# Shaibk/Matrix-FHE-GPU

Hardware: AMD Instinct MI355X
Metric: forward-NTT/s (N=2^16, L RNS limbs) (higher is better)
Workload: dtype u64; 1 GPU; batched forward negacyclic NTT (phantom convention), N=2^16, L=8 x 50-bit primes, batch=1024 per GPU; N=65536, limbs=8, batch_per_gpu=1024, arith=f64, parallelism=residue-batch shard x1 (no collective)

## Files before the change

matrix-fhe-gpu_amd/csrc/ntt_kernels.hpp:

```cpp
#pragma once
#include <type_traits>

#include "ntt_arith.hpp"

#ifndef MFHE_NTT_CPOL_IN
#define MFHE_NTT_CPOL_IN 0
#endif
#ifndef MFHE_NTT_CPOL_OUT
#define MFHE_NTT_CPOL_OUT 18
#endif
#ifndef MFHE_NTT_CPOL_MID_LD
#define MFHE_NTT_CPOL_MID_LD 0
#endif
#ifndef MFHE_NTT_CPOL_MID_ST
#define MFHE_NTT_CPOL_MID_ST 0
#endif
#ifndef MFHE_NTT_U64_INV_TWPRE
#define MFHE_NTT_U64_INV_TWPRE 1
#endif
#ifndef MFHE_NTT_COL_DMA
#define MFHE_NTT_COL_DMA 1
#endif

namespace mfhe {

struct TwSrcF {
    const double* p;
    __device__ __forceinline__ double get(size_t i) const { return p[i]; }
};
struct TwSrcU {
    const uint64_t* w;
    const uint64_t* ws;
    __device__ __forceinline__ ulonglong2 get(size_t i) const {
#ifdef MFHE_EXP_TWCONST
        return make_ulonglong2((uint64_t)i * 0x9E3779B97F4A7C15ull >> 6, (uint64_t)i * 0xC2B2AE3D27D4EB4Full);
#endif
        return make_ulonglong2(w[i], ws[i]);
    }
};

template <class TS>
struct PassArgs {
    uint64_t* data;
    TS tw;
    TS twist;
    TS ninv;
    const LimbConst* limbs;
    const uint64_t* qraw;
    int qstride;
    uint64_t batch;
    int nl, start_limb;
    int logN, s0;
    uint32_t nblocks;
};

__device__ __forceinline__ uint32_t xcd_remap(uint32_t b, uint32_t nb) {
    const uint32_t q = nb >> 3, r = nb & 7, x = b & 7, s = b >> 3;
    return (x < r ? x * (q + 1) : r * (q + 1) + (x - r) * q) + s;
}

template <int LOG_G, int LOG_R>
struct Geo {
    static constexpr int G = 1 << LOG_G;
    static constexpr int R = 1 << LOG_R;
    static constexpr int TG = G / R;
    static constexpr int NR = (LOG_G + LOG_R - 1) / LOG_R;
    static constexpr int GS = G + G / 16 + 1;
    __host__ __device__ static constexpr int HB(int r) { return LOG_G - 1 - r * LOG_R; }
    __host__ __device__ static constexpr int WL(int r) { return (HB(r) - LOG_R + 1) > 0 ? (HB(r) - LOG_R + 1) : 0; }
    __device__ __forceinline__ static uint32_t g_of(int r, uint32_t tau, uint32_t k) {
        const int wl = WL(r);
        return ((tau >> wl) << (wl + LOG_R)) | (k << wl) | (tau & ((1u << wl) - 1));
    }
    __device__ __forceinline__ static uint32_t pad(uint32_t g) { return g + (g >> 4); }
};

__device__ __forceinline__ uint32_t brev_bits(uint32_t x, int bits) { return __brev(x) >> (32 - bits); }

template <int I, int N, class F>
__device__ __forceinline__ void static_for(F&& f) {
    if constexpr (I < N) {
        f(std::integral_constant<int, I>{});
        static_for<I + 1, N>(f);
    }
}

template <int R, int BB, bool LAST, class A, class T, class TWF>
__device__ __forceinline__ void u60_inv_stage(const A& ar, T (&x)[R], TWF&& tw, typename A::Tw wn) {
    constexpr int half = 1 << BB;
    static_for<0, R>([&](auto kc) {
        constexpr int k = decltype(kc)::value;
        if constexpr (!(k & half)) {
            constexpr int e0 = U60InvBounds<R>::after(k, BB);
            constexpr int e = e0 == 3 ? 0 : e0;
            if constexpr (e0 == 3) {
                x[k] = ar.template red<3>(x[k]);
                x[k + half] = ar.template red<3>(x[k + half]);
            }
            const auto w = tw(k);
            ar.template gs_b<e>(x[k], x[k + half], w);
            if constexpr (LAST) x[k] = ar.mulmod(x[k], wn);
        }
    });
}

template <class A>
__device__ __forceinline__ uint64_t inv_out(const A& ar, typename A::T x) {
    if constexpr (kLazyU60<A>) return ar.canon_inv(x);
    else return ar.canon(x);
}

template <int R, int N, class A, class T>
__device__ __forceinline__ void u60_inv_round_end(const A& ar, T (&x)[R]) {
    static_for<0, R>([&](auto kc) {
        constexpr int k = decltype(kc)::value;
        x[k] = ar.template red<U60InvBounds<R>::after(k, N)>(x[k]);
    });
}

struct TileLoc {
    uint64_t* base;
    size_t twoff;
    uint32_t off0;
    uint64_t hi;
    int mod;
    bool active;
};

template <int LOG_G, int NG, bool COLS, bool UNI>
__device__ __forceinline__ TileLoc tile_loc(uint64_t* data, uint64_t batch, int nl, int start_limb, int logN, int s0,
                                            uint32_t lb, uint32_t gl) {
    const int logS = logN - s0 - LOG_G;
    const int log_gpp = logS + s0;
    const uint32_t npl = (uint32_t)(batch * (uint64_t)nl);
    uint32_t v;
    uint64_t hi, lo;
    if constexpr (COLS) {
        constexpr int LOG_NG = __builtin_ctz(NG);
        const int log_tpp = log_gpp - LOG_NG, log_ct = logS - LOG_NG;
        v = lb >> log_tpp;
        const uint32_t tile = lb & ((1u << log_tpp) - 1);
        hi = tile >> log_ct;
        lo = ((uint64_t)(tile & ((1u << log_ct) - 1)) << LOG_NG) + gl;
    } else if constexpr (UNI) {
        const uint64_t g0 = (uint64_t)lb * NG;
        v = (uint32_t)(g0 >> log_gpp);
        const uint64_t rem = (g0 & ((1ull << log_gpp) - 1)) + gl;
        hi = rem >> logS;
        lo = rem & ((1ull << logS) - 1);
    } else {
        const uint64_t gid = (uint64_t)lb * NG + gl;
        v = (uint32_t)(gid >> log_gpp);
        const uint64_t rem = gid & ((1ull << log_gpp) - 1);
        hi = rem >> logS;
        lo = rem & ((1ull << logS) - 1);
    }
    TileLoc t;
    t.active = v < npl;
    if (!t.active) v = 0;
    const uint32_t bt = (uint32_t)batch;
    const int l = (int)(v / bt);
    const uint64_t b = v - (uint32_t)l * bt;
    t.mod = start_limb + l;
    t.base = data + ((b * (uint64_t)nl + (uint64_t)l) << logN);
    t.twoff = (size_t)t.mod << logN;
    t.hi = hi;
    t.off0 = (uint32_t)((hi << (logN - s0)) | lo);
    return t;
}

constexpr int kPackUnitBytes = 1664;
constexpr int kPackRowBytes = 2048;

template <class A, class TS, int LOG_G, int LOG_R, int NG, bool COLS, bool INV, bool IN_RAW, bool OUT_RAW,
          bool TWIST, bool BREV, bool UNI, bool PACK = false>
struct NttPass {
    static_assert(!PACK || (LOG_G == 8 && LOG_R == 4 && NG == 16 && UNI && !INV && !TWIST && !BREV &&
                            (COLS ? (OUT_RAW && !IN_RAW) : (IN_RAW && !OUT_RAW))),
                  "PACK: forward N = 2^16 two-pass plan only");
    static constexpr bool COL_DMA = MFHE_NTT_COL_DMA && COLS && !INV && !IN_RAW && UNI && !TWIST &&
                                    (1 << LOG_G) * NG * 8 == 32768 && NG % 2 == 0;
    static constexpr bool PACK_OUT = PACK && COLS;
    static constexpr bool PACK_IN = PACK && !COLS;
    using Gm = Geo<LOG_G, LOG_R>;
    using T = typename A::T;
    using Tw = typename A::Tw;
    static constexpr int R = Gm::R, TG = Gm::TG, NR = Gm::NR, GS = Gm::GS;
    static constexpr int NT = NG * TG;
    static constexpr size_t LDS_BYTES = (NR > 1 || BREV) ? (size_t)NG * GS * sizeof(uint64_t) : 0;
    static constexpr int r_load = (INV && COLS) ? (NR - 1) : 0;
    static constexpr int r_store = (!INV && COLS) ? (NR - 1) : 0;

    const PassArgs<TS>& a;
    uint32_t gl, tau;
    int s0, logS;

    __device__ __forceinline__ explicit NttPass(const PassArgs<TS>& args) : a(args) {
        const uint32_t t = threadIdx.x;
        gl = COLS ? (t % NG) : (t / TG);
        tau = COLS ? (t / NG) : (t % TG);
        s0 = COLS ? 0 : a.logN - LOG_G;
        logS = a.logN - s0 - LOG_G;
    }
    __device__ __forceinline__ uint32_t jidx(const TileLoc& L, uint32_t g) const { return L.off0 | (g << logS); }
    __device__ __forceinline__ TileLoc locate(uint32_t lb) const {
        return tile_loc<LOG_G, NG, COLS, UNI>(a.data, a.batch, a.nl, a.start_limb, a.logN, s0, lb, gl);
    }
    static constexpr int kCpolLd = IN_RAW ? MFHE_NTT_CPOL_MID_LD : MFHE_NTT_CPOL_IN;
    static constexpr int kCpolSt = OUT_RAW ? MFHE_NTT_CPOL_MID_ST : MFHE_NTT_CPOL_OUT;

    __device__ __forceinline__ void load(const TileLoc& L, uint64_t (&raw)[R]) const {
        if constexpr (COL_DMA) return;
        if constexpr (PACK_IN) {
            const uint32_t rb = (uint32_t)(L.hi >> 4);
            const char* base = (const char*)L.base + (size_t)(16 * rb) * kPackRowBytes;
#pragma unroll
            for (int s = 0; s < 7; ++s) {
                const uint32_t q = threadIdx.x + NT * s;
                ulonglong2 v = make_ulonglong2(0, 0);
                if (s < 6 || q < 16 * kPackUnitBytes / 16) {
                    const uint32_t t = q / 104, w = q - 104 * t;
                    v = *(const ulonglong2*)(base + (w >> 3) * kPackRowBytes + t * 128 + (w & 7) * 16);
                }
                raw[2 * s] = v.x;
                raw[2 * s + 1] = v.y;
            }
            return;
        }
        if constexpr (UNI && kCpolLd != 0) {
            const __amdgpu_buffer_rsrc_t rs = __builtin_amdgcn_make_buffer_rsrc(L.base, 0, 0x7FFFFFFF, 0x00020000);
#pragma unroll
            for (int k = 0; k < R; ++k)
                raw[k] = __builtin_bit_cast(uint64_t, __builtin_amdgcn_raw_buffer_load_b64(
                                                          rs, (int)(jidx(L, Gm::g_of(r_load, tau, k)) * 8u), 0, kCpolLd));
        } else {
#pragma unroll
            for (int k = 0; k < R; ++k) {
#ifdef MFHE_EXP_SKIP
                if (IN_RAW && k >= 12) { raw[k] = 0; continue; }
#endif
                raw[k] = L.base[jidx(L, Gm::g_of(r_load, tau, k))];
            }
        }
    }

    __device__ __forceinline__ void compute_store(const TileLoc& L, const uint64_t (&raw)[R], uint64_t* lds) const {
        uint64_t* my_lds = lds + (size_t)gl * GS;
        LimbConst lc;
        if (a.limbs) {
            lc = a.limbs[L.mod];
        } else {
            lc.q = a.qraw[(size_t)L.mod * a.qstride];
            lc.qf = (double)lc.q;
            lc.qinv = 1.0 / lc.qf;
        }
        const A ar(lc);
        const size_t twoff = L.twoff;
        const uint32_t tau_ = tau;

        T x[R];
        if constexpr (COL_DMA) {
            typedef __attribute__((address_space(3))) void* lds_vp;
            constexpr int CPR = NG / 2;
            const uint32_t w = threadIdx.x >> 6, lane = threadIdx.x & 63;
            const char* tile = (const char*)(L.base + (L.off0 - gl));
            __syncthreads();
#pragma unroll
            for (int i = 0; i < 32768 / (NT * 16); ++i) {
                const uint32_t q = (i * (NT / 64) + w) * 64 + lane;
                const char* src = tile + (size_t)(q / CPR) * ((size_t)8 << (a.logN - LOG_G)) + (q % CPR) * 16;
                __builtin_amdgcn_global_load_lds((const void*)src,
                                                 (lds_vp)((char*)lds + (size_t)(i * (NT / 64) + w) * 1024), 16, 0,
                                                 kCpolLd);
            }
            asm volatile("s_waitcnt vmcnt(0)" ::: "memory");
            __syncthreads();
#pragma unroll
            for (int k = 0; k < R; ++k) x[k] = A::from_u64(lds[(size_t)Gm::g_of(r_load, tau_, k) * NG + gl]);
        } else if constexpr (PACK_IN) {
            __syncthreads();
            ulonglong2* img = (ulonglong2*)lds;
#pragma unroll
            for (int s = 0; s < 7; ++s) {
                const uint32_t q = threadIdx.x + NT * s;
                if (s < 6 || q < 16 * kPackUnitBytes / 16) img[q] = make_ulonglong2(raw[2 * s], raw[2 * s + 1]);
            }
            __syncthreads();
            const uint32_t C = threadIdx.x, t = C >> 4, c = C & 15;
            const char* ub = (const char*)lds + t * kPackUnitBytes;
            uint64_t w[13];
#pragma unroll
            for (int s = 0; s < 4; ++s) {
                const ulonglong2 v = *(const ulonglong2*)(ub + c * 64 + 16 * s);
                w[2 * s] = v.x;
                w[2 * s + 1] = v.y;
            }
#pragma unroll
            for (int s = 0; s < 2; ++s) {
                const ulonglong2 v = *(const ulonglong2*)(ub + 1024 + c * 32 + 16 * s);
                w[8 + 2 * s] = v.x;
                w[9 + 2 * s] = v.y;
            }
            w[12] = *(const uint32_t*)(ub + 1536 + c * 4);
            __syncthreads();
#pragma unroll
            for (int i = 0; i < 16; ++i) {
                const uint64_t lo = (w[i >> 1] >> (32 * (i & 1))) & 0xFFFFFFFFull;
                const uint64_t mid = (w[8 + (i >> 2)] >> (16 * (i & 3))) & 0xFFFFull;
                const uint64_t top = (w[12] >> (2 * i)) & 3ull;
                lds[(size_t)i * GS + Gm::pad(C)] = lo | (mid << 32) | (top << 48);
            }
            __syncthreads();
#pragma unroll
            for (int k = 0; k < R; ++k) x[k] = A::from_u64(my_lds[Gm::pad(Gm::g_of(0, tau_, k))]);
        } else {
#pragma unroll
            for (int k = 0; k < R; ++k) {
                x[k] = IN_RAW ? A::from_raw(raw[k]) : A::from_u64(raw[k]);
                if constexpr (TWIST && !INV) x[k] = ar.mulmod(x[k], a.twist.get(twoff + jidx(L, Gm::g_of(r_load, tau_, k))));
            }
        }

        auto exchange = [&](auto rf, auto rt, bool brev_pos) {
            constexpr int r_from = decltype(rf)::value, r_to = decltype(rt)::value;
            __syncthreads();
#pragma unroll
            for (int k = 0; k < R; ++k) {
                uint32_t g = Gm::g_of(r_from, tau_, k);
                if (brev_pos) g = brev_bits(g, LOG_G);
                my_lds[Gm::pad(g)] = A::to_raw(x[k]);
            }
            __syncthreads();
#pragma unroll
            for (int k = 0; k < R; ++k) x[k] = A::from_raw(my_lds[Gm::pad(Gm::g_of(r_to, tau_, k))]);
        };

        constexpr bool kTwPre = INV && !COLS && kIsU64<A> && MFHE_NTT_U64_INV_TWPRE;
        Tw wpre[kTwPre ? R / 2 : 1];
        if constexpr (kTwPre) {
            constexpr int r = NR - 1, wl = Gm::WL(r), bit = wl;
            const int s = s0 + (LOG_G - 1 - bit);
            const uint64_t twb = twoff + (1ull << s) + (L.hi << (LOG_G - 1 - bit)) + ((uint64_t)(tau_ >> wl) << (LOG_R - 1));
#pragma unroll
            for (int m = 0; m < R / 2; ++m) wpre[m] = a.tw.get(twb + (uint64_t)m);
        }
        if constexpr (INV && !COLS && (NR > 1 || BREV))
            exchange(std::integral_constant<int, 0>{}, std::integral_constant<int, NR - 1>{}, BREV);

        auto stage = [&](auto rc, auto bc) {
            constexpr int r = decltype(rc)::value, bb = decltype(bc)::value;
            constexpr int hb = Gm::HB(r), wl = Gm::WL(r);
            constexpr int bit = wl + bb;
            if constexpr (bit <= hb) {
                const int s = s0 + (LOG_G - 1 - bit);
                constexpr int half = 1 << bb;
                const uint64_t tau_hi = tau_ >> wl;
                const uint64_t twb =
                    twoff + (1ull << s) + (L.hi << (LOG_G - 1 - bit)) + (tau_hi << (LOG_R - 1 - bb));
                if constexpr (!INV) {
                    constexpr int fb = (LOG_R - 1 < hb - wl) ? LOG_R - 1 : hb - wl;
                    constexpr bool first = bb == fb && (r > 0 || IN_RAW);
                    static_assert(!kLazyU60<A> || LOG_R <= 4, "U60 bound: at most 4 stages between reductions");
#pragma unroll
                    for (int k = 0; k < R; ++k) {
                        if (k & half) continue;
                        const Tw w = a.tw.get(twb + (uint64_t)(k >> (bb + 1)));
                        if constexpr (first) ar.ct_first(x[k], x[k + half], w);
                        else ar.ct(x[k], x[k + half], w);
                    }
                } else {
                    constexpr int ri = NR - 1 - r;
                    constexpr int first = (Gm::HB(NR - 1) < LOG_R - 1 ? Gm::HB(NR - 1) : LOG_R - 1) + 1;
                    constexpr int e = ri == 0 ? bb : first + (ri - 1) * LOG_R + bb;
                    if constexpr (kLazyU60<A>) {
                        if (s == 0) {
                            const Tw wn = a.ninv.get((size_t)L.mod);
                            const Tw w1 = a.tw.get(twoff + 1);
                            u60_inv_stage<R, bb, true>(ar, x, [&](int) { return w1; }, wn);
                        } else {
                            u60_inv_stage<R, bb, false>(ar, x, [&](int k) {
                                if constexpr (kTwPre && r == NR - 1 && bb == 0) return wpre[k >> 1];
                                else return a.tw.get(twb + (uint64_t)(k >> (bb + 1)));
                            }, Tw{});
                        }
                    } else if (s == 0) {
                        const Tw wn = a.ninv.get((size_t)L.mod);
                        const Tw w1 = a.tw.get(twoff + 1);
#pragma unroll
                        for (int k = 0; k < R; ++k) {
                            if (k & half) continue;
                            T u = x[k], vv = x[k + half];
                            ar.gs_lazy(u, vv, w1);
                            x[k] = ar.mulmod(u, wn);
                            x[k + half] = vv;
                        }
                    } else {
#pragma unroll
                        for (int k = 0; k < R; ++k) {
                            if (k & half) continue;
                            Tw w;
                            if constexpr (kTwPre && r == NR - 1 && bb == 0) w = wpre[k >> 1];
                            else w = a.tw.get(twb + (uint64_t)(k >> (bb + 1)));
                            if constexpr (e % 2 == 0) ar.gs_lazy(x[k], x[k + half], w);
                            else ar.gs(x[k], x[k + half], w);
                        }
                    }
                }
            }
        };

        if constexpr (!INV) {
            static_for<0, NR>([&](auto rc) {
                constexpr int r = decltype(rc)::value;
                if constexpr (r > 0) {
                    exchange(std::integral_constant<int, r - 1>{}, rc, false);
#pragma unroll
                    for (int k = 0; k < R; ++k) x[k] = ar.round_reduce(x[k]);
                }
                static_for<0, LOG_R>([&](auto bi) {
                    stage(rc, std::integral_constant<int, LOG_R - 1 - decltype(bi)::value>{});
                });
            });
        } else {
            static_for<0, NR>([&](auto ri) {
                constexpr int r = NR - 1 - decltype(ri)::value;
                if constexpr (r < NR - 1)
                    exchange(std::integral_constant<int, r + 1>{}, std::integral_constant<int, r>{}, false);
                static_for<0, LOG_R>([&](auto bi) { stage(std::integral_constant<int, r>{}, bi); });
                if constexpr (kLazyU60<A>) {
                    constexpr int hb = Gm::HB(r), wl = Gm::WL(r);
                    constexpr int nexec = (hb - wl + 1) < LOG_R ? (hb - wl + 1) : LOG_R;
                    if constexpr (r > 0 || OUT_RAW) u60_inv_round_end<R, nexec>(ar, x);
                }
            });
        }

        if constexpr (!INV && !COLS && (NR > 1 || BREV))
            exchange(std::integral_constant<int, NR - 1>{}, std::integral_constant<int, 0>{}, BREV);
        if constexpr (PACK_OUT) {
            uint32_t lo[16], mid[8] = {}, top = 0;
#pragma unroll
            for (int k = 0; k < 16; ++k) {
                const uint64_t u = ar.canon(x[k]);
                lo[k] = (uint32_t)u;
                const uint32_t hi = (uint32_t)(u >> 32);
                mid[k >> 1] |= (hi & 0xFFFFu) << (16 * (k & 1));
                top |= (hi >> 16) << (2 * k);
            }
            __syncthreads();
            char* ub = (char*)lds + tau_ * kPackUnitBytes;
            uint4* plo = (uint4*)(ub + gl * 64);
            uint4* pmid = (uint4*)(ub + 1024 + gl * 32);
#pragma unroll
            for (int s = 0; s < 4; ++s) plo[s] = make_uint4(lo[4 * s], lo[4 * s + 1], lo[4 * s + 2], lo[4 * s + 3]);
#pragma unroll
            for (int s = 0; s < 2; ++s) pmid[s] = make_uint4(mid[4 * s], mid[4 * s + 1], mid[4 * s + 2], mid[4 * s + 3]);
            *(uint32_t*)(ub + 1536 + gl * 4) = top;
            __syncthreads();
            if (L.active) {
                const uint4* src = (const uint4*)lds;
                char* dst = (char*)L.base + (size_t)(L.off0 & ~15u) * 8;
                for (uint32_t q = threadIdx.x; q < 16 * kPackUnitBytes / 16; q += NT) {
                    const uint32_t m = q >> 3, rb = m / 13, j = m - 13 * rb;
                    *(uint4*)(dst + (size_t)(16 * rb + j) * kPackRowBytes + (q & 7) * 16) = src[q];
                }
            }
            return;
        }
        if (L.active) {
            if constexpr (UNI && kCpolSt != 0) {
                const __amdgpu_buffer_rsrc_t rs = __builtin_amdgcn_make_buffer_rsrc(L.base, 0, 0x7FFFFFFF, 0x00020000);
#pragma unroll
                for (int k = 0; k < R; ++k) {
                    const uint32_t g = Gm::g_of(r_store, tau_, k);
                    T y = x[k];
                    if constexpr (TWIST && INV) y = ar.mulmod(y, a.twist.get(twoff + jidx(L, g)));
                    const uint64_t o = OUT_RAW ? ar.raw_out(y) : INV ? inv_out(ar, y) : ar.canon(y);
                    __builtin_amdgcn_raw_buffer_store_b64(__builtin_bit_cast(__attribute__((ext_vector_type(2))) unsigned, o),
                                                          rs, (int)(jidx(L, g) * 8u), 0, kCpolSt);
                }
            } else {
#pragma unroll
                for (int k = 0; k < R; ++k) {
                    const uint32_t g = Gm::g_of(r_store, tau_, k);
                    T y = x[k];
                    if constexpr (TWIST && INV) y = ar.mulmod(y, a.twist.get(twoff + jidx(L, g)));
#ifdef MFHE_EXP_SKIP
                    if (OUT_RAW && k >= 12) continue;
#endif
                    L.base[jidx(L, g)] = OUT_RAW ? ar.raw_out(y) : INV ? inv_out(ar, y) : ar.canon(y);
                }
            }
        }
    }
};

template <class P, bool PF, class TS>
__device__ __forceinline__ void pass_loop(const PassArgs<TS>& a, uint64_t* lds) {
    const P p(a);
    const uint32_t nb = a.nblocks;
    uint32_t lt = blockIdx.x;
    if (lt >= nb) return;
    TileLoc L = p.locate(xcd_remap(lt, nb));
    uint64_t raw[P::R];
    p.load(L, raw);
    while (true) {
        const uint32_t nlt = lt + gridDim.x;
        const bool more = nlt < nb;
        TileLoc Ln;
        uint64_t nraw[PF ? P::R : 1];
        if constexpr (PF) {
            if (more) {
                Ln = p.locate(xcd_remap(nlt, nb));
                p.load(Ln, nraw);
            }
        }
        p.compute_store(L, raw, lds);
        if (!more) break;
        lt = nlt;
        if constexpr (PF) {
            L = Ln;
            for (int k = 0; k < P::R; ++k) raw[k] = nraw[k];
        } else {
            L = p.locate(xcd_remap(lt, nb));
            p.load(L, raw);
        }
    }
}

#ifndef MFHE_NTT_MIN_WG_CU
#define MFHE_NTT_MIN_WG_CU 1
#endif
constexpr int min_waves_per_simd(int nt) {
    return (MFHE_NTT_MIN_WG_CU * nt / 256) < 1 ? 1 : (MFHE_NTT_MIN_WG_CU * nt / 256);
}

#ifndef MFHE_NTT_U64_BLOCK_W4
#define MFHE_NTT_U64_BLOCK_W4 0
#endif
template <class A, bool COLS>
constexpr int pass_min_waves(int nt) {
    return (MFHE_NTT_U64_BLOCK_W4 && kIsU64<A> && !COLS && nt <= 256) ? 4 : min_waves_per_simd(nt);
}

template <class A, class TS, int LOG_G, int LOG_R, int NG, bool COLS, bool INV, bool IN_RAW, bool OUT_RAW,
          bool TWIST, bool BREV, bool UNI, bool PF, bool PACK = false>
__global__ __launch_bounds__(NG * (1 << (LOG_G - LOG_R)), (pass_min_waves<A, COLS>(NG * (1 << (LOG_G - LOG_R)))))
void ntt_pass_kernel(PassArgs<TS> a) {
    extern __shared__ __attribute__((aligned(16))) uint64_t lds[];
    pass_loop<NttPass<A, TS, LOG_G, LOG_R, NG, COLS, INV, IN_RAW, OUT_RAW, TWIST, BREV, UNI, PACK>, PF>(a, lds);
}

}
```

Before: 2.849 million NTT/s.

## Prefetch per-round twiddles before LDS exchange and use lighter LDS-only barriers

Generalises the inverse-only twiddle prefetch so that, in the row (block) pass, the twiddles for up to four stages of the next radix round are loaded into registers before the shared-memory exchange. Global twiddle latency can then overlap the exchange barrier. It also swaps __syncthreads in the row-pass exchange for an inline s_waitcnt lgkmcnt(0) plus s_barrier, or only a waitcnt when the block fits in one wavefront, which skips waiting on outstanding global memory operations. The costs are higher register pressure from the prefetch array and correctness that now depends on hand-written barrier semantics.

New measurement: 2.864 million NTT/s (median of 6 runs). No clear change (+0.6%).

```diff
diff --git a/matrix-fhe-gpu_amd/csrc/ntt_kernels.hpp b/matrix-fhe-gpu_amd/csrc/ntt_kernels.hpp
--- a/matrix-fhe-gpu_amd/csrc/ntt_kernels.hpp
+++ b/matrix-fhe-gpu_amd/csrc/ntt_kernels.hpp
@@ -17,6 +17,15 @@
 #endif
 #ifndef MFHE_NTT_U64_INV_TWPRE
 #define MFHE_NTT_U64_INV_TWPRE 1
+#endif
+#ifndef MFHE_NTT_U64_BLOCK_TWPRE
+#define MFHE_NTT_U64_BLOCK_TWPRE 4
+#endif
+#ifndef MFHE_NTT_F64_BLOCK_TWPRE
+#define MFHE_NTT_F64_BLOCK_TWPRE 4
+#endif
+#ifndef MFHE_NTT_BLOCK_LDS_SYNC
+#define MFHE_NTT_BLOCK_LDS_SYNC 1
 #endif
 #ifndef MFHE_NTT_COL_DMA
 #define MFHE_NTT_COL_DMA 1
@@ -191,6 +200,29 @@
     static constexpr int r_load = (INV && COLS) ? (NR - 1) : 0;
     static constexpr int r_store = (!INV && COLS) ? (NR - 1) : 0;
 
+    static constexpr bool LDS_ONLY_SYNC = !COLS && MFHE_NTT_BLOCK_LDS_SYNC;
+    __device__ __forceinline__ static void lds_sync_before_write() {
+        if constexpr (!LDS_ONLY_SYNC) __syncthreads();
+        else if constexpr (NT <= 64) asm volatile("" ::: "memory");
+        else asm volatile("s_waitcnt lgkmcnt(0)\n\ts_barrier" ::: "memory");
+    }
+    __device__ __forceinline__ static void lds_sync_before_read() {
+        if constexpr (!LDS_ONLY_SYNC) __syncthreads();
+        else if constexpr (NT <= 64) asm volatile("s_waitcnt lgkmcnt(0)" ::: "memory");
+        else asm volatile("s_waitcnt lgkmcnt(0)\n\ts_barrier" ::: "memory");
+    }
+
+    static constexpr bool BLOCK = !COLS && (INV ? OUT_RAW : IN_RAW);
+    static constexpr int TWPRE = !BLOCK ? 0 : kIsU64<A> ? MFHE_NTT_U64_BLOCK_TWPRE : MFHE_NTT_F64_BLOCK_TWPRE;
+    static constexpr int TWPRE_ENTRY = (INV && !COLS && kIsU64<A> && MFHE_NTT_U64_INV_TWPRE && TWPRE < 1) ? 1 : TWPRE;
+    __host__ __device__ static constexpr int nexec(int r) {
+        return (Gm::HB(r) - Gm::WL(r) + 1) < LOG_R ? (Gm::HB(r) - Gm::WL(r) + 1) : LOG_R;
+    }
+    __host__ __device__ static constexpr bool tw_pre(int r, int bb) {
+        const int n = INV ? (r == NR - 1 ? TWPRE_ENTRY : TWPRE) : (r > 0 ? TWPRE : 0);
+        return bb < nexec(r) && (INV ? bb : nexec(r) - 1 - bb) < n;
+    }
+
     const PassArgs<TS>& a;
     uint32_t gl, tau;
     int s0, logS;
@@ -323,27 +355,36 @@
 
         auto exchange = [&](auto rf, auto rt, bool brev_pos) {
             constexpr int r_from = decltype(rf)::value, r_to = decltype(rt)::value;
-            __syncthreads();
+            lds_sync_before_write();
 #pragma unroll
             for (int k = 0; k < R; ++k) {
                 uint32_t g = Gm::g_of(r_from, tau_, k);
                 if (brev_pos) g = brev_bits(g, LOG_G);
                 my_lds[Gm::pad(g)] = A::to_raw(x[k]);
             }
-            __syncthreads();
+            lds_sync_before_read();
 #pragma unroll
             for (int k = 0; k < R; ++k) x[k] = A::from_raw(my_lds[Gm::pad(Gm::g_of(r_to, tau_, k))]);
         };
 
-        constexpr bool kTwPre = INV && !COLS && kIsU64<A> && MFHE_NTT_U64_INV_TWPRE;
-        Tw wpre[kTwPre ? R / 2 : 1];
-        if constexpr (kTwPre) {
-            constexpr int r = NR - 1, wl = Gm::WL(r), bit = wl;
+        auto tw_base = [&](auto rc, auto bc) -> uint64_t {
+            constexpr int r = decltype(rc)::value, bb = decltype(bc)::value;
+            constexpr int wl = Gm::WL(r), bit = wl + bb;
             const int s = s0 + (LOG_G - 1 - bit);
-            const uint64_t twb = twoff + (1ull << s) + (L.hi << (LOG_G - 1 - bit)) + ((uint64_t)(tau_ >> wl) << (LOG_R - 1));
-#pragma unroll
-            for (int m = 0; m < R / 2; ++m) wpre[m] = a.tw.get(twb + (uint64_t)m);
-        }
+            return twoff + (1ull << s) + (L.hi << (LOG_G - 1 - bit)) + ((uint64_t)(tau_ >> wl) << (LOG_R - 1 - bb));
+        };
+        Tw wp[LOG_R][R / 2];
+        auto tw_prefetch = [&](auto rc) {
+            static_for<0, LOG_R>([&](auto bc) {
+                constexpr int r = decltype(rc)::value, bb = decltype(bc)::value;
+                if constexpr (tw_pre(r, bb)) {
+                    const uint64_t twb = tw_base(rc, bc);
+#pragma unroll
+                    for (int m = 0; m < (R >> (bb + 1)); ++m) wp[bb][m] = a.tw.get(twb + (uint64_t)m);
+                }
+            });
+        };
+        if constexpr (INV) tw_prefetch(std::integral_constant<int, NR - 1>{});
         if constexpr (INV && !COLS && (NR > 1 || BREV))
             exchange(std::integral_constant<int, 0>{}, std::integral_constant<int, NR - 1>{}, BREV);
 
@@ -354,9 +395,11 @@
             if constexpr (bit <= hb) {
                 const int s = s0 + (LOG_G - 1 - bit);
                 constexpr int half = 1 << bb;
-                const uint64_t tau_hi = tau_ >> wl;
-                const uint64_t twb =
-                    twoff + (1ull << s) + (L.hi << (LOG_G - 1 - bit)) + (tau_hi << (LOG_R - 1 - bb));
+                const uint64_t twb = tw_base(rc, bc);
+                auto tw_at = [&](int m) -> Tw {
+                    if constexpr (tw_pre(r, bb)) return wp[bb][m];
+                    else return a.tw.get(twb + (uint64_t)m);
+                };
                 if constexpr (!INV) {
                     constexpr int fb = (LOG_R - 1 < hb - wl) ? LOG_R - 1 : hb - wl;
                     constexpr bool first = bb == fb && (r > 0 || IN_RAW);
@@ -364,7 +407,7 @@
 #pragma unroll
                     for (int k = 0; k < R; ++k) {
                         if (k & half) continue;
-                        const Tw w = a.tw.get(twb + (uint64_t)(k >> (bb + 1)));
+                        const Tw w = tw_at(k >> (bb + 1));
                         if constexpr (first) ar.ct_first(x[k], x[k + half], w);
                         else ar.ct(x[k], x[k + half], w);
                     }
@@ -378,10 +421,7 @@
                             const Tw w1 = a.tw.get(twoff + 1);
                             u60_inv_stage<R, bb, true>(ar, x, [&](int) { return w1; }, wn);
                         } else {
-                            u60_inv_stage<R, bb, false>(ar, x, [&](int k) {
-                                if constexpr (kTwPre && r == NR - 1 && bb == 0) return wpre[k >> 1];
-                                else return a.tw.get(twb + (uint64_t)(k >> (bb + 1)));
-                            }, Tw{});
+                            u60_inv_stage<R, bb, false>(ar, x, [&](int k) { return tw_at(k >> (bb + 1)); }, Tw{});
                         }
                     } else if (s == 0) {
                         const Tw wn = a.ninv.get((size_t)L.mod);
@@ -398,9 +438,7 @@
 #pragma unroll
                         for (int k = 0; k < R; ++k) {
                             if (k & half) continue;
-                            Tw w;
-                            if constexpr (kTwPre && r == NR - 1 && bb == 0) w = wpre[k >> 1];
-                            else w = a.tw.get(twb + (uint64_t)(k >> (bb + 1)));
+                            const Tw w = tw_at(k >> (bb + 1));
                             if constexpr (e % 2 == 0) ar.gs_lazy(x[k], x[k + half], w);
                             else ar.gs(x[k], x[k + half], w);
                         }
@@ -413,6 +451,7 @@
             static_for<0, NR>([&](auto rc) {
                 constexpr int r = decltype(rc)::value;
                 if constexpr (r > 0) {
+                    tw_prefetch(rc);
                     exchange(std::integral_constant<int, r - 1>{}, rc, false);
 #pragma unroll
                     for (int k = 0; k < R; ++k) x[k] = ar.round_reduce(x[k]);
@@ -424,8 +463,10 @@
         } else {
             static_for<0, NR>([&](auto ri) {
                 constexpr int r = NR - 1 - decltype(ri)::value;
-                if constexpr (r < NR - 1)
+                if constexpr (r < NR - 1) {
+                    tw_prefetch(std::integral_constant<int, r>{});
                     exchange(std::integral_constant<int, r + 1>{}, std::integral_constant<int, r>{}, false);
+                }
                 static_for<0, LOG_R>([&](auto bi) { stage(std::integral_constant<int, r>{}, bi); });
                 if constexpr (kLazyU60<A>) {
                     constexpr int hb = Gm::HB(r), wl = Gm::WL(r);
```
